# spcl/EBCC

Measured on AMD Instinct MI355X. Metric: fp32 GB/s encode+decode, 721x1440 ERA5 frames MAX_ERROR=0.5, higher is better.
Workload: dtype f32; 1 GPU; 256-frame batch 721x1440 fp32 per GPU, base_cr=30 MAX_ERROR=0.5 (BASELINE configs[1]); frames_per_gpu=256, parallelism=frames sharded over 1 GPU(s), no collective, hw_queues=4, encode_slices=3

## Files before the change

### ebcc_amd/csrc/j2k.hip

```cpp
#include <algorithm>
#include <cstring>
#include <vector>

#include "../../include/ebcc_hip.h"
#include "engine.hpp"
#include "j2k.hpp"

namespace ebcc {

bool j2k_create(ebcc_hip_ctx *ctx)
{
    J2kBuffers *jb = new J2kBuffers();
    ctx->j2k = jb;
    const int period = ctx->tile_period;
    std::vector<std::vector<J2kBlock>> tile_blocks((size_t) period);
    int stride = 0;
    for (int k = 0; k < period; k++) {
        jb->geoms.push_back(make_j2k_geom(ctx->height, ctx->width, tile_blocks[(size_t) k], k * ctx->height));
        stride = std::max(stride, jb->geoms.back().nblocks);
    }
    for (J2kGeom &t : jb->geoms) { t.period = period; t.stride = stride; }
    jb->geom = jb->geoms[0];
    const J2kGeom &g = jb->geom;
    const size_t n_pix = ctx->n_pix, F = ctx->max_frames;
// ... 19 lines not shown
    jb->SYM = nullptr;
    {
        const char *e = getenv("EBCC_T1_TWO_PHASE");
        jb->sym_rows = kJ2kSymRows;
        if (const char *r = getenv("EBCC_HIP_SYM_ROWS")) jb->sym_rows = std::max(1, std::min(kJ2kSymRows, atoi(r)));
        if (!e || atoi(e)) ok &= (jb->SYM = ctx_alloc<uint8_t>(ctx, groups * (size_t) ((jb->sym_rows + 1) & ~1) * 1024 + 256)) != nullptr;
    }
    ok &= (jb->seglen = ctx_alloc<uint16_t>(ctx, groups * (size_t) kJ2kSegCount * 64)) != nullptr;
    ok &= (jb->lanerows = ctx_alloc<uint32_t>(ctx, groups * 64)) != nullptr;
    ok &= (jb->qplane = (int *) ctx_alloc<int32_t>(ctx, groups * 64)) != nullptr;
    ok &= (jb->lastnp = (int *) ctx_alloc<int32_t>(ctx, groups * 64)) != nullptr;
    ok &= (jb->T1S = ctx_alloc<unsigned long long>(ctx, groups * kT1StateWords * 64)) != nullptr;
    ok &= (jb->blkmax = (int *) ctx_alloc<int32_t>(ctx, groups * 64)) != nullptr;
    ok &= (jb->numbps = (int *) ctx_alloc<int32_t>(ctx, groups * 64)) != nullptr;
    ok &= (jb->totalpasses = (int *) ctx_alloc<int32_t>(ctx, groups * 64)) != nullptr;
    ok &= (jb->cblk_len = (int *) ctx_alloc<int32_t>(ctx, groups * 64)) != nullptr;
    ok &= (jb->npass = (int *) ctx_alloc<int32_t>(ctx, groups * 64)) != nullptr;
    ok &= (jb->cand_cr = ctx_alloc<float>(ctx, F * 2)) != nullptr;
    ok &= (jb->cand_out = (int *) ctx_alloc<int32_t>(ctx, F * 6)) != nullptr;
    ok &= (jb->cand_npass = (int *) ctx_alloc<int32_t>(ctx, 2 * F * (size_t) stride)) != nullptr;
    ok &= (jb->cand_sel = (int *) ctx_alloc<int32_t>(ctx, F)) != nullptr;
    ok &= (jb->have_rate = (int *) ctx_alloc<int32_t>(ctx, F)) != nullptr;
    ok &= (jb->rate_path = (int *) ctx_alloc<int32_t>(ctx, F * 1536 * 3)) != nullptr;
    ok &= (jb->rate_path_n = (int *) ctx_alloc<int32_t>(ctx, 2 * F)) != nullptr;
    {
        int nodes = 0;
        for (const J2kGeom &t : jb->geoms) nodes = std::max(nodes, t.tree_nodes);
        J2kBuffers::RateCache &rc = jb->rate_cache;
        rc.nodes_cap = (nodes + 3) & ~3;
        rc.cap = stride * kJ2kMaxPasses;
        rc.ok = jb->rate_path_n ? jb->rate_path_n + F : nullptr;
        ok &= (rc.mnmx = ctx_alloc<double>(ctx, F * 2)) != nullptr;
        ok &= (rc.mval = (short *) ctx_alloc<uint16_t>(ctx, F * (size_t) rc.nodes_cap)) != nullptr;
        ok &= (rc.off = (int *) ctx_alloc<int32_t>(ctx, F * (size_t) (stride + 1))) != nullptr;
        ok &= (rc.crate = ctx_alloc<uint16_t>(ctx, F * (size_t) rc.cap)) != nullptr;
        ok &= (rc.cdisto = ctx_alloc<double>(ctx, F * (size_t) rc.cap)) != nullptr;
    }
    ok &= (jb->rates = (int *) ctx_alloc<int32_t>(ctx, groups * 64 * kJ2kMaxPasses)) != nullptr;
    ok &= (jb->disto = ctx_alloc<double>(ctx, groups * 64 * kJ2kMaxPasses)) != nullptr;
    ok &= (jb->cblk_bytes = ctx_alloc<uint8_t>(ctx, groups * 64 * kJ2kCblkBytes)) != nullptr;
    ok &= (jb->stream = ctx_alloc<uint8_t>(ctx, F * jb->stream_cap)) != nullptr;
    ok &= (jb->dec_table = (int *) ctx_alloc<int32_t>(ctx, groups * 64 * 4)) != nullptr;
    ok &= (jb->dec_order = (int *) ctx_alloc<int32_t>(ctx, groups * 64 + 128)) != nullptr;
    ok &= (jb->mq_order = (int *) ctx_alloc<int32_t>(ctx, groups * 64 + 256)) != nullptr;
    ok &= (jb->jf = (J2kFrame *) ctx_alloc<uint8_t>(ctx, sizeof(J2kFrame) * F)) != nullptr;
    ok &= (jb->partial = ctx_alloc<double>(ctx, F * kPartials)) != nullptr;
    ok &= (jb->partial_u = ctx_alloc<unsigned long long>(ctx, F * kPartials)) != nullptr;
    if (!ok) return false;
    poison_alloc(jb->cblk_bytes, groups * 64 * kJ2kCblkBytes);
    poison_alloc(jb->stream, F * jb->stream_cap);
    if (stride >= 65535) { set_error("too many code-blocks"); return false; }
    std::vector<uint16_t> map((size_t) period * n_pix, 0);
    std::vector<J2kBlock> blocks((size_t) period * (size_t) stride, J2kBlock{});
    for (int k = 0; k < period; k++) {
        const std::vector<J2kBlock> &tb = tile_blocks[(size_t) k];
        std::copy(tb.begin(), tb.end(), blocks.begin() + (size_t) k * (size_t) stride);
        for (size_t b = 0; b < tb.size(); b++)
            for (int y = 0; y < tb[b].h; y++)
                for (int x = 0; x < tb[b].w; x++) map[(size_t) k * n_pix + (size_t) (tb[b].y + y) * g.W + tb[b].x + x] = (uint16_t) b;
    }
    hipStream_t s = ctx->stream;
    EBCC_HIP_CHECK(hipMemcpyAsync(jb->d_geom, jb->geoms.data(), sizeof(J2kGeom) * (size_t) period, hipMemcpyHostToDevice, s));
    EBCC_HIP_CHECK(hipMemcpyAsync(jb->d_blocks, blocks.data(), sizeof(J2kBlock) * blocks.size(), hipMemcpyHostToDevice, s));
    EBCC_HIP_CHECK(hipMemcpyAsync(jb->d_blkmap, map.data(), map.size() * sizeof(uint16_t), hipMemcpyHostToDevice, s));
    EBCC_HIP_CHECK(hipHostMalloc(&ctx->h_jf, sizeof(J2kFrame) * F));
    EBCC_HIP_CHECK(hipHostMalloc((void **) &ctx->h_table, sizeof(int) * 4 * total));
    EBCC_HIP_CHECK(hipMemsetAsync(jb->jf, 0, sizeof(J2kFrame) * F, s));
    EBCC_HIP_CHECK(hipMemsetAsync(jb->rate_path_n, 0, sizeof(int) * 2 * F, s));
    wait_stream(s);
    return true;
}

void j2k_destroy(ebcc_hip_ctx *ctx)
{
    delete static_cast<J2kBuffers *>(ctx->j2k);
    ctx->j2k = nullptr;
    if (ctx->stream2) { hipStreamSynchronize(ctx->stream2); hipStreamDestroy(ctx->stream2); ctx->stream2 = nullptr; }
}

namespace {

struct BitReader {
    const uint8_t *p, *end;
    unsigned buf = 0;
    int ct = 0;
    int bit()
    {
        if (ct == 0) {
            buf = (buf << 8) & 0xFFFF;
            ct = buf == 0xFF00 ? 7 : 8;
            if (p < end) buf |= *p++;
// ... 470 lines not shown
```

### ebcc_amd/csrc/j2k.hpp

```cpp
#pragma once

#include <vector>

#include "../../include/ebcc_hip.h"
#include "common.hpp"
#include "residual.hpp"

namespace ebcc {

constexpr int kJ2kRes = 6;
constexpr int kJ2kBands = 3 * kJ2kRes - 2;
constexpr int kJ2kMaxPlanes = 26;
constexpr int kJ2kMaxPasses = 3 * kJ2kMaxPlanes;
constexpr int kJ2kCblkBytes = 16 * 1024;
constexpr int kT1StateWords = 66 + 4 * 64;

struct J2kBand {
    int res, orient, level;
    int x0, y0, x1, y1;
    int offx, offy;
    int ncw, nch;
    int first_block;
    int expn, mant, numbps;
    float step_enc, step_dec;
// ... 88 lines not shown
    unsigned long long *T1S;
    int *blkmax;
    int *numbps;
    int *totalpasses;
    int *cblk_len;
    int *rates;
    double *disto;
    int *npass;
    float *cand_cr;
    int *cand_out;
    int *cand_npass;
    int *cand_sel;
    int *have_rate;
    int *rate_path;
    int *rate_path_n;
    struct RateCache {
        int *ok;
        double *mnmx;
        short *mval;
        int *off;
        unsigned short *crate;
        double *cdisto;
        int nodes_cap, cap;
    } rate_cache;
    uint8_t *cblk_bytes;
    uint8_t *stream;
    size_t stream_cap;
    int32_t *V;
    int *dec_table;
    int *dec_order;
    int *mq_order;
    J2kFrame *jf;
    FrameState *fs;
    double *partial;
    unsigned long long *partial_u;
};

enum T1Kernel { T1_ENCODE = 0, T1_MQ = 1, T1_RESUME = 2, T1_DECODE = 3 };
int t1_lanes_per_wave(int kernel, int total_blocks = 0);

J2kGeom make_j2k_geom(int H, int W, std::vector<J2kBlock> &blocks, int ty0 = 0);

struct J2kWindow {
    int row0, col0, rows, cols;
    int rx0[kJ2kRes], rx1[kJ2kRes], ry0[kJ2kRes], ry1[kJ2kRes];
    int band[kJ2kBands][4];
// ... 58 lines not shown
```

### ebcc_amd/csrc/j2k_analysis.hip

```cpp
#include <array>
#include <mutex>
#include <cmath>
#include <cstdlib>
#include <vector>

#include "j2k.hpp"
#include "t1_core.hpp"
#include "t1_device.hpp"

namespace ebcc {

static int ceildivpow2(int a, int b) { return (int) (((long long) a + (1ll << b) - 1) >> b); }
static int floorlog2i(int a) { int l = 0; while (a > 1) { a >>= 1; l++; } return l; }

static const double kNormsReal[4][10] = {
    {1.000, 1.965, 4.177, 8.403, 16.90, 33.84, 67.69, 135.3, 270.6, 540.9},
    {2.022, 3.989, 8.355, 17.04, 34.27, 68.63, 137.3, 274.6, 549.0},
    {2.022, 3.989, 8.355, 17.04, 34.27, 68.63, 137.3, 274.6, 549.0},
    {2.080, 3.865, 8.307, 17.18, 34.71, 69.59, 139.3, 278.6, 557.2}};

int t1_lanes_per_wave(int kernel, int total_blocks)
{
    int t[4] = {64, 64, 4, 2};
    if (const char *e = getenv("EBCC_T1_LPW")) {
// ... 1101 lines not shown
};
__device__ inline Tier1Lane tier1_lane(int gid, int total, const int *blkmax, const J2kGeom *geom, const J2kBlock *blocks, const FrameState *fs)
{
    Tier1Lane l{gid, 0, 0, 0, 0, 0, false};
    if (gid >= total) return l;
    const int nb = geom->stride;
    l.frame = gid / nb;
    if (fs[l.frame].const_field) return l;
    const J2kBlock blk = j2k_frame_blocks(geom, blocks, l.frame)[gid - l.frame * nb];
    const int m = blkmax[gid];
    l.P = m ? (31 - __clz(m)) + 1 - 6 : 0;
    l.w = blk.w; l.h = blk.h;
    l.orient = j2k_frame_geom(geom, l.frame).bands[blk.band].orient;
    l.live = l.P > 0;
    return l;
}

struct ScanOutDev {
    unsigned char *vp, *sp;
    std::uint16_t *lens;
    uint32_t lane8;
    __device__ void visp_row(unsigned char *b, int row, unsigned long long v) const { *(unsigned long long *) (b + ((uint32_t) row * 512u + lane8)) = v; }
    __device__ void visp(int p, int y, unsigned long long m) const { visp_row(vp, p * 64 + y, m); }
    __device__ void sps_or(int y, unsigned long long n) const { *(unsigned long long *) (sp + ((uint32_t) y * 512u + lane8)) |= n; }
    __device__ void len(int seg, uint32_t n) const { lens[(uint32_t) seg * 64u] = (std::uint16_t) n; }
};
__global__ __launch_bounds__(64) void k_t1_scan(const unsigned long long *BP, const unsigned long long *SUF, const unsigned long long *SGN,
                                                 unsigned long long *SPS, unsigned long long *VISP, const int *blkmax, int *numbps,
                                                 int *totalpasses, int *cblk_len, std::uint16_t *seglen, const J2kGeom *geom,
                                                 const J2kBlock *blocks, const FrameState *fs, int total)
{
    const size_t grp = blockIdx.x;
    const int gid = (int) (grp * 64) + (int) threadIdx.x;
    const Tier1Lane l = tier1_lane(gid, total, blkmax, geom, blocks, fs);
    if (gid < total) { numbps[gid] = l.P; totalpasses[gid] = l.live ? 3 * l.P - 2 : 0; cblk_len[gid] = 0; }
    if (!l.live) return;
    const uint32_t lane8 = threadIdx.x * 8u;
    DevMasks M{(const unsigned char *) (BP + grp * kJ2kMaxPlanes * 64 * 64), (const unsigned char *) (SUF + grp * (kJ2kMaxPlanes + 2) * 64 * 64),
               (const unsigned char *) (SGN + grp * 64 * 64), (unsigned char *) (VISP + grp * kJ2kMaxPlanes * 64 * 64), lane8};
    ScanOutDev out{M.visp, (unsigned char *) (SPS + grp * 64 * 64), seglen + grp * kJ2kSegCount * 64 + threadIdx.x, lane8};
    t1::scan_block(M, out, l.P, l.w, l.h, l.orient);
}

__global__ __launch_bounds__(64) void k_t1_rowoffs(std::uint16_t *seglen, uint32_t *lanerows, const int *blkmax, J2kFrame *jf,
                                                    const J2kGeom *geom, const J2kBlock *blocks, const FrameState *fs, int total,
                                                    uint32_t sym_rows)
{
    const size_t grp = blockIdx.x;
    const int gid = (int) (grp * 64) + (int) threadIdx.x;
    const Tier1Lane l = tier1_lane(gid, total, blkmax, geom, blocks, fs);
    std::uint16_t *L = seglen + grp * kJ2kSegCount * 64 + threadIdx.x;
    uint32_t off = 0;
    if (l.live) {
        const int nstr = (l.h + 3) >> 2;
        for (int seg0 = t1::seg_index(l.P - 1, 2, 0) & ~15; seg0 < kJ2kSegCount; seg0 += 16) {
            if (!t1::seg_valid(l.P, nstr, t1::seg_plane(seg0), t1::seg_type(seg0), 0)) continue;
            uint32_t n[16];
#pragma unroll
            for (int k = 0; k < 16; k++) n[k] = k < nstr ? L[(uint32_t) (seg0 + k) * 64u] : 0u;
#pragma unroll
            for (int k = 0; k < 16; k++)
                if (k < nstr) { L[(uint32_t) (seg0 + k) * 64u] = (std::uint16_t) off; off += t1::seg_rows(n[k]); }
        }
    }
// ... 339 lines not shown
{
    const int f = blockIdx.x * blockDim.x + threadIdx.x;
    if (f < n) jf[f].overflow = 0;
}

void launch_j2k_tier1(const J2kBuffers &jb, int n_frames, hipStream_t s, bool single_kernel)
{
    const J2kGeom &g = jb.geom;
    const FrameState *fs = jb.fs;
    const int total = n_frames * g.stride;
    const size_t groups = ((size_t) total + 63) / 64;
    EBCC_HIP_CHECK(hipMemsetAsync(jb.SPS, 0, groups * 64 * 64 * sizeof(unsigned long long), s));
    timing_begin("t1_encode", s);
    if (!jb.SYM || single_kernel) {
        EBCC_HIP_CHECK(hipMemsetAsync(jb.T1S, 0, groups * kT1StateWords * 64 * sizeof(unsigned long long), s));
        int lpw = getenv("EBCC_T1_LPW") ? t1_lanes_per_wave(T1_ENCODE) : 32;
        unsigned t1_grid = (unsigned) ceil_div(total, lpw);
        hipLaunchKernelGGL(k_t1_encode, dim3(t1_grid), dim3(64), 0, s, jb.T1S, jb.BP, jb.SGN, jb.SPS, jb.blkmax, jb.numbps,
                           jb.totalpasses, jb.cblk_len, jb.rates, jb.cblk_bytes, jb.ckpt, jb.VISP, jb.d_geom,
                           jb.d_blocks, fs, jb.jf, total, lpw);
    } else {
        EBCC_HIP_CHECK(hipMemsetAsync(jb.seglen, 0, groups * (size_t) kJ2kSegCount * 64 * sizeof(std::uint16_t), s));
        timing_begin("t1_symbols", s);
        hipLaunchKernelGGL(k_t1_scan, dim3((unsigned) groups), dim3(64), 0, s, jb.BP, jb.SUF, jb.SGN, jb.SPS, jb.VISP, jb.blkmax, jb.numbps,
                           jb.totalpasses, jb.cblk_len, jb.seglen, jb.d_geom, jb.d_blocks, fs, total);
        hipLaunchKernelGGL(k_t1_rowoffs, dim3((unsigned) groups), dim3(64), 0, s, jb.seglen, jb.lanerows, jb.blkmax, jb.jf, jb.d_geom, jb.d_blocks,
                           fs, total, (uint32_t) jb.sym_rows);
        hipLaunchKernelGGL(k_t1_emit, dim3((unsigned) groups, kJ2kMaxPlanes), dim3(64), 0, s, jb.BP, jb.SUF, jb.SGN, jb.VISP, jb.blkmax, jb.SYM,
                           jb.seglen, jb.lanerows, jb.d_geom, jb.d_blocks, fs, total, (uint32_t) jb.sym_rows);
        timing_end("t1_symbols", s);
        if (getenv("EBCC_HIP_T1_STATS")) {
            std::vector<uint32_t> tot((size_t) total);
            EBCC_HIP_CHECK(hipMemcpyAsync(tot.data(), jb.lanerows, sizeof(uint32_t) * (size_t) total, hipMemcpyDeviceToHost, s));
            wait_stream(s);
            uint32_t mx = 0; double sum = 0, wsum = 0;
            for (size_t g0 = 0; g0 < (size_t) total; g0 += 64) {
                uint32_t wm = 0;
                for (size_t i = g0; i < std::min((size_t) total, g0 + 64); i++) { wm = std::max(wm, tot[i]); sum += tot[i]; }
                wsum += wm; mx = std::max(mx, wm);
            }
            fprintf(stderr, "ebcc-mi355x tier-1: %zu groups, rows of 16 decisions: per code-block mean %.0f, per wave mean %.0f max %u (cap %d)\n", groups,
                    sum / (double) total, wsum / (double) groups, mx, jb.sym_rows);
        }
        timing_begin("t1_mq", s);
        const int *order = nullptr;
        if (!getenv("EBCC_HIP_MQ_NATURAL_ORDER")) {
            int *counters = jb.mq_order + groups * 64;
// ... 65 lines not shown
            const float e2 = (i < dn) ? e1_2 + (((i == 0 ? o2 : o2_3) + o2) * kD) : e1_2 + ((2 * o2_3) * kD);
            b[(size_t) i * W] = e2 * invK;
            if (i < dn) b[(size_t) (sn + i) * W] = o2 * kK;
        }
        E_1 = E0; O_1 = O0;
        o1_2 = o1; e1_2 = e1;
        o2_3 = o2;
        e_in = e_nx; o_in = o_nx;
    }
}

void launch_j2k_analysis(const float *data, const J2kBuffers &jb, int n_frames, hipStream_t s)
{
    const FrameState *fs = jb.fs;
    const J2kGeom &g = jb.geom;
    const size_t n_pix = (size_t) g.W * g.H;
    const int total = n_frames * g.stride;
    hipLaunchKernelGGL(k_jf_reset, dim3(ceil_div(n_frames, 64)), dim3(64), 0, s, jb.jf, n_frames);
    const bool fwd_top = g.period == 1 && g.ry0[kJ2kRes - 1] % 2 == 0 && g.rh[kJ2kRes - 2] >= 2 &&
                         g.rh[kJ2kRes - 1] - g.rh[kJ2kRes - 2] >= 1;
    if (!fwd_top) hipLaunchKernelGGL(k_scale_shift, dim3(128, n_frames), dim3(256), 0, s, data, jb.B, n_pix, fs);
    EBCC_HIP_CHECK(hipMemsetAsync(jb.rate_path_n, 0, sizeof(int) * (size_t) n_frames, s));
    EBCC_HIP_CHECK(hipMemsetAsync(jb.rate_cache.ok, 0, sizeof(int) * (size_t) n_frames, s));
    EBCC_HIP_CHECK(hipMemsetAsync(jb.lastnp, 0xFF, sizeof(int) * (size_t) total, s));
    timing_begin("j2k_dwt_fwd", s);
    for (int r = kJ2kRes - 1; r >= 1; r--) {
        if (fwd_top && r == kJ2kRes - 1) {
            const int pieces = std::max(1, std::min(8, g.rh[r - 1] / 16));
            hipLaunchKernelGGL(k_j2k_cols_fwd_top, dim3(ceil_div(g.rw[r], kFwdT), n_frames, pieces), dim3(kFwdT), 0, s, data, jb.B, jb.d_geom, fs);
        } else
        dwt_cols<true>(jb.B, jb, r, n_frames, fs, nullptr, s);
        if (g.rw[r] > 1) dwt_rows<true>(jb.B, nullptr, jb, r, n_frames, fs, nullptr, s);
    }
    timing_end("j2k_dwt_fwd", s);
    hipLaunchKernelGGL(k_quantize, dim3((unsigned) (((size_t) total + 63) / 64)), dim3(256), 0, s, jb.B, jb.Q6, jb.BP, jb.SGN, jb.SUF, jb.blkmax,
                       jb.d_geom, jb.d_blocks, fs, total);
    launch_j2k_tier1(jb, n_frames, s, false);
    EBCC_HIP_LAUNCH_CHECK();
}

int j2k_first_fused(const J2kBuffers &jb)
{
    const J2kGeom &g = jb.geom;
    auto fusable = [&](int r) {
        return g.period == 1 && g.ry0[r] % 2 == 0 && g.rw[r - 1] >= 2 && g.rh[r - 1] >= 1 &&
               (r == kJ2kRes - 1 ? ceil_div(g.rw[r - 1], kL5Pairs) <= kPartials : jb.B2 != nullptr);
// ... 123 lines not shown
```

### ebcc_amd/csrc/j2k_rate.hip

```cpp
#include <cfloat>
#include <cmath>
#include <cstdlib>
#include <mutex>

#include "j2k.hpp"
#include "t1_core.hpp"
#include "t1_device.hpp"

namespace ebcc {

int j2k_inverse_dwt(float *B, const int32_t *V, const float *data, const J2kBuffers &jb, int n_frames, const FrameState *fs,
                    const int *active, hipStream_t s, int keep_field, const J2kWindow *win = nullptr, float *win_out = nullptr);

namespace {

constexpr int kMainHeaderBytes = 135;
constexpr int kRateTrieNodes = 1536;
#ifndef EBCC_RATE_THREADS
#define EBCC_RATE_THREADS 512
#endif
constexpr int kRateThreads = EBCC_RATE_THREADS;
constexpr int kWriteThreads = 256;

__device__ inline int floorlog2d(int a) { return a > 1 ? 31 - __clz(a) : 0; }
// ... 456 lines not shown
    }
    if (wl == 0) atomicAdd(s_sum, body + count);
    __syncthreads();
    const int total = *s_sum;
    __syncthreads();
    return total;
}

__global__ __launch_bounds__(kRateThreads) void k_rate(const int *__restrict__ numbps, const int *__restrict__ totalpasses,
                                                        const int *__restrict__ rates, const double *__restrict__ disto,
                                                        int *__restrict__ npass_out, const J2kGeom *geom, J2kFrame *jf,
                                                        const FrameState *fs, const int *active, int pass_capacity,
                                                        int *__restrict__ path_bytes, int *__restrict__ path_n,
                                                        const float *cand_cr, int *cand_out, size_t cand_stride, const int *have_rate,
                                                        J2kBuffers::RateCache cache)
{
    extern __shared__ unsigned char lds_raw[];
    __shared__ int s_sum, s_changed;
#ifdef EBCC_RATE_PROFILE
    const long long t_start = wall_clock64();
#endif
    __shared__ double s_min[kRateThreads / 64], s_max[kRateThreads / 64];
    __shared__ double s_td[5];
    __shared__ int s_ti[5], s_nun, s_list[64];
    const int frame = blockIdx.x, lane = threadIdx.x;
    if ((active && !active[frame]) || fs[frame].const_field) return;
    const bool candidate = cand_cr != nullptr;
    const int slot = candidate ? (int) blockIdx.y : 0;
    const float cr_in = candidate ? cand_cr[2 * frame + slot] : jf[frame].cr;
    if (candidate ? !(cr_in > 0.0f) : (have_rate && have_rate[frame])) return;
    if (candidate) npass_out += (size_t) slot * cand_stride;
    const bool record = !candidate;
    const J2kGeom &g = j2k_frame_geom(geom, frame);
    const int gid0 = frame * g.stride;
    RateLds L;
    L.carve(lds_raw, g.nblocks, g.tree_nodes);
#ifdef EBCC_RATE_PROFILE
    long long t_s[5] = {0, 0, 0, 0, 0};
    t_s[0] = wall_clock64() - t_start;
#endif
    __shared__ int s_cached;
    if (lane == 0) s_cached = __hip_atomic_load(&cache.ok[frame], __ATOMIC_ACQUIRE, __HIP_MEMORY_SCOPE_AGENT);
    __syncthreads();
    const bool cached = s_cached != 0;
    short *const c_mval = cache.mval + (size_t) frame * cache.nodes_cap;
    int *const c_off = cache.off + (size_t) frame * (size_t) (g.stride + 1);
    unsigned short *const c_rate = cache.crate + (size_t) frame * (size_t) cache.cap;
// ... 126 lines not shown
    if ((lane & 63) == 0) { s_min[lane >> 6] = mn; s_max[lane >> 6] = mx; }
    __syncthreads();
    for (int i = 0; i < kRateThreads / 64; i++) { mn = s_min[i] < mn ? s_min[i] : mn; mx = s_max[i] > mx ? s_max[i] : mx; }
    if (record) {
        __threadfence();
        __syncthreads();
        if (lane == 0) {
            cache.mnmx[2 * frame] = mn; cache.mnmx[2 * frame + 1] = mx;
            if (pt.lds) { __threadfence(); __hip_atomic_store(&cache.ok[frame], 1, __ATOMIC_RELEASE, __HIP_MEMORY_SCOPE_AGENT); }
        }
    }
    }

#ifdef EBCC_RATE_PROFILE
    long long t_setup = wall_clock64() - t_start, t_ml = 0, t_sz = 0, t_replay_end = 0, t_tail = 0, t_loop_end = 0; int n_it = 0, n_real = 0, n_replayed = 0, n_tail = 0;
#define RP_T0 const long long rp0 = wall_clock64()
#define RP_ADD(acc) acc += wall_clock64() - rp0
#else
#define RP_T0
#define RP_ADD(acc)
#endif
    double good = -1;
    bool converged = false;
    if (rate > 0.0f) {
        const long long maxlen = (long long) ceil((double) rate);
        double lo = mn, hi = mx, thresh = 0, stable = 0, prev = -1;
        bool lo_seen = false, hi_seen = false;
        int bytes_lo = 0, bytes_hi = 0;
        int *const trie = path_bytes + (size_t) frame * kRateTrieNodes * 3;
        const int known = path_n[frame];
        int n_nodes = known;
        int cur = known > 0 ? 0 : -1, parent = -1, pdir = 0;
        bool lo_from_rec = false, hi_from_rec = false;
        for (int i = 0; i < 128; i++) {
            thresh = (lo + hi) / 2;
            if (i > 0 && thresh == prev) break;
            prev = thresh;
            if (cur >= 0) {
#ifdef EBCC_RATE_PROFILE
                n_replayed++;
#endif
                const int bytes = trie[3 * cur];
                const int f = (long long) bytes <= maxlen;
                if (f) { hi = thresh; stable = thresh; bytes_hi = bytes; hi_from_rec = true; hi_seen = false; }
                else { lo = thresh; bytes_lo = bytes; lo_from_rec = true; lo_seen = false; }
                parent = cur; pdir = f;
                const int nxt = trie[3 * cur + 1 + f];
                cur = nxt > 0 ? nxt : -1;
                continue;
            }
#ifdef EBCC_RATE_PROFILE
            if (!t_replay_end) t_replay_end = wall_clock64();
#endif
            if (hi_from_rec) { make_layer<kRateThreads>(g, L, totalpasses, pt, gid0, hi, lane, p_hi); hi_seen = true; hi_from_rec = false; }
            if (lo_from_rec) { make_layer<kRateThreads>(g, L, totalpasses, pt, gid0, lo, lane, p_lo); lo_seen = true; lo_from_rec = false; }
            { RP_T0; make_layer<kRateThreads>(g, L, totalpasses, pt, gid0, thresh, lane, p_cur, frozen); RP_ADD(t_ml); }
            if (lane == 0) s_nun = 0;
            int at_lo = lo_seen, at_hi = hi_seen;
            for (int b = lane; b < g.nblocks; b += kRateThreads) {
                if (frozen[b]) continue;
                if (p_cur[b] != p_lo[b] || p_cur[g.nblocks + b] != p_lo[g.nblocks + b]) at_lo = 0;
                if (p_cur[b] != p_hi[b] || p_cur[g.nblocks + b] != p_hi[g.nblocks + b]) at_hi = 0;
            }
            at_lo = __syncthreads_and(at_lo);
            at_hi = __syncthreads_and(at_hi);
            int bytes;
            if (at_lo) bytes = bytes_lo;
            else if (at_hi) bytes = bytes_hi;
            else { RP_T0; bytes = sized(); RP_ADD(t_sz); }
#ifdef EBCC_RATE_PROFILE
            n_it++; n_real += (at_lo || at_hi) ? 0 : s_changed;
#endif
            const bool fits = (long long) bytes <= maxlen;
            if (record && n_nodes < kRateTrieNodes && (parent >= 0 || n_nodes == 0)) {
                if (lane == 0) {
                    trie[3 * n_nodes] = bytes; trie[3 * n_nodes + 1] = 0; trie[3 * n_nodes + 2] = 0;
                    if (parent >= 0) trie[3 * parent + 1 + pdir] = n_nodes;
                    path_n[frame] = n_nodes + 1;
                }
                parent = n_nodes++; pdir = fits;
            } else {
                parent = -1;
            }
            if (fits) bytes_hi = bytes; else bytes_lo = bytes;
            if (fits) { hi = thresh; stable = thresh; hi_seen = true; } else { lo = thresh; lo_seen = true; }
            unsigned long long *end = fits ? p_hi : p_lo;
            int same = lo_seen && hi_seen;
            for (int b = lane; b < g.nblocks; b += kRateThreads) {
                if (frozen[b]) continue;
                end[b] = p_cur[b]; end[g.nblocks + b] = p_cur[g.nblocks + b];
                if (lo_seen && hi_seen && p_lo[b] == p_hi[b] && p_lo[g.nblocks + b] == p_hi[g.nblocks + b]) frozen[b] = 1;
                else {
                    same = 0;
                    const int k = atomicAdd(&s_nun, 1);
                    if (k < 64) s_list[k] = b;
                }
            }
            if (__syncthreads_and(same)) { converged = true; break; }
            if (lo_seen && hi_seen && s_nun <= 64) {
                RP_T0;
                if (lane < 64) {
                    const int nb = g.nblocks, b = lane < s_nun ? s_list[lane] : -1;
                    double tlo = lo, thi = hi, tprev = prev, tstable = stable, tthresh = thresh;
                    int ti = i, tn = n_nodes, tparent = parent, tpdir = pdir, status = 0;
                    int from = 0, n_in = 0;
                    unsigned long long c0 = 0, c1 = 0;
                    if (b >= 0) {
                        const unsigned long long d0 = p_lo[b] ^ p_hi[b], d1 = p_lo[nb + b] ^ p_hi[nb + b];
                        from = d0 ? __builtin_ctzll(d0) : (d1 ? 64 + __builtin_ctzll(d1) : 0);
                        if (from > 0) {
                            c0 = from >= 64 ? p_lo[b] : p_lo[b] & ((1ull << from) - 1ull);
                            c1 = from > 64 ? p_lo[nb + b] & ((1ull << (from - 64)) - 1ull) : 0ull;
                            n_in = c1 ? 128 - __builtin_clzll(c1) : (c0 ? 64 - __builtin_clzll(c0) : 0);
                        }
                    }
                    double a_lo = -DBL_MAX, b_lo = DBL_MAX, a_hi = -DBL_MAX, b_hi = DBL_MAX;
                    if (b >= 0) {
                        if (pt.lds) {
                            walk_interval<true>(pt, totalpasses, gid0, b, p_lo[b], p_lo[nb + b], from, n_in, tlo, thi, a_lo, b_lo);
                            walk_interval<true>(pt, totalpasses, gid0, b, p_hi[b], p_hi[nb + b], from, n_in, tlo, thi, a_hi, b_hi);
                        } else {
                            walk_interval<false>(pt, totalpasses, gid0, b, p_lo[b], p_lo[nb + b], from, n_in, tlo, thi, a_lo, b_lo);
                            walk_interval<false>(pt, totalpasses, gid0, b, p_hi[b], p_hi[nb + b], from, n_in, tlo, thi, a_hi, b_hi);
                        }
                    }
                    (void) c0; (void) c1;
                    for (int j = i + 1; j < 128; j++) {
                        const double t = (tlo + thi) / 2;
                        if (t == tprev) { tthresh = t; break; }
                        const int all_lo = __all(b < 0 || (t >= a_lo && t < b_lo));
                        const int all_hi = __all(b < 0 || (t >= a_hi && t < b_hi));
                        if (!all_lo && !all_hi) { status = 1; break; }
                        tthresh = t; tprev = t; ti = j;
                        const int bytes = all_lo ? bytes_lo : bytes_hi;
                        const bool fits = (long long) bytes <= maxlen;
                        if (record && tn < kRateTrieNodes && (tparent >= 0 || tn == 0)) {
                            if (lane == 0) {
                                trie[3 * tn] = bytes; trie[3 * tn + 1] = 0; trie[3 * tn + 2] = 0;
                                if (tparent >= 0) trie[3 * tparent + 1 + tpdir] = tn;
                                path_n[frame] = tn + 1;
                            }
                            tparent = tn++; tpdir = fits;
                        } else {
                            tparent = -1;
                        }
                        if (fits) { thi = t; tstable = t; } else { tlo = t; }
                    }
                    if (lane == 0) {
                        s_td[0] = tlo; s_td[1] = thi; s_td[2] = tprev; s_td[3] = tstable; s_td[4] = tthresh;
                        s_ti[0] = ti; s_ti[1] = tn; s_ti[2] = tparent; s_ti[3] = tpdir; s_ti[4] = status;
                    }
                }
                __syncthreads();
                lo = s_td[0]; hi = s_td[1]; prev = s_td[2]; stable = s_td[3]; thresh = s_td[4];
                i = s_ti[0]; n_nodes = s_ti[1]; parent = s_ti[2]; pdir = s_ti[3];
                const int status = s_ti[4];
                __syncthreads();
                RP_ADD(t_tail);
#ifdef EBCC_RATE_PROFILE
                n_tail++;
#endif
                if (status == 0) break;
            }
        }
        good = stable == 0 ? thresh : stable;
    }
#ifdef EBCC_RATE_PROFILE
    t_loop_end = wall_clock64();
#endif
    if (!converged) make_layer<kRateThreads>(g, L, totalpasses, pt, gid0, good, lane);
    const int body = sized();
    for (int b = lane; b < g.nblocks; b += kRateThreads) npass_out[gid0 + b] = L.npass[b];
    if (lane == 0 && candidate) {
        int *o = cand_out + (size_t) (2 * frame + slot) * 3;
        o[0] = body; o[1] = kMainHeaderBytes + 12 + 2 + body + 2; o[2] = (int) (rate > 0.0f ? ceil((double) rate) : 0);
    }
    if (lane == 0 && !candidate) {
        jf[frame].body_bytes = body;
        jf[frame].stream_bytes = kMainHeaderBytes + 12 + 2 + body + 2;
        jf[frame].maxlen = (int) (rate > 0.0f ? ceil((double) rate) : 0);
#ifdef EBCC_RATE_PROFILE
        if (frame == 0) printf("k_rate frame0 setup: entry %lld, trees %lld, offsets %lld, tables %lld us\n", t_s[0] / 100, t_s[1] / 100, t_s[2] / 100, t_s[3] / 100);
        if (frame == 0) printf("k_rate frame0: setup %lld us, %d replayed steps until %lld us, make_layer %lld us, sized %lld us, computed iterations %d (real sizings %d), tail %lld us in %d visits, loop ends at %lld us, total %lld us\n",
                               t_setup / 100, n_replayed, t_replay_end ? (t_replay_end - t_start) / 100 : -1, t_ml / 100, t_sz / 100, n_it, n_real, t_tail / 100, n_tail,
                               (t_loop_end - t_start) / 100, (wall_clock64() - t_start) / 100);
#endif
    }
}

__device__ inline void put16(uint8_t *&p, unsigned v) { *p++ = (uint8_t) (v >> 8); *p++ = (uint8_t) v; }
__device__ inline void put32(uint8_t *&p, unsigned v) { put16(p, v >> 16); put16(p, v & 0xFFFFu); }

__global__ __launch_bounds__(kWriteThreads) void k_write(const int *__restrict__ numbps, const int *__restrict__ rates,
                                                         const int *__restrict__ npass_in, const uint8_t *__restrict__ cblk_bytes,
                                                         uint8_t *__restrict__ stream, size_t stream_cap, const J2kGeom *geom,
                                                         J2kFrame *jf, const FrameState *fs, const int *active)
{
    extern __shared__ unsigned char lds_raw[];
    __shared__ int s_hdr[kJ2kRes], s_body[kJ2kRes], s_off[kJ2kRes + 1];
    const int frame = blockIdx.x, lane = threadIdx.x;
    if ((active && !active[frame]) || fs[frame].const_field) return;
    const J2kGeom &g = j2k_frame_geom(geom, frame);
    const int gid0 = frame * g.stride;
    RateLds L;
    L.carve(lds_raw, g.nblocks, g.tree_nodes);
    trees_static<kWriteThreads>(g, L, numbps, gid0, lane);
    for (int b = lane; b < g.nblocks; b += kWriteThreads) L.npass[b] = (short) npass_in[gid0 + b];
    __syncthreads();
// ... 749 lines not shown
```

### ebcc_amd/csrc/t1_core.hpp

```cpp
#pragma once

#include <cstdint>
#include <type_traits>

#if defined(__HIPCC__)
#define T1_HD __host__ __device__ inline
#else
#define T1_HD inline
#endif
#ifndef T1_STAT
#define T1_STAT(i)
#endif

namespace ebcc {
namespace t1 {

typedef unsigned long long u64;

enum { CTX_ZC0 = 0, CTX_SC0 = 9, CTX_MAG0 = 14, CTX_AGG = 17, CTX_UNI = 18, NCTX = 19 };
constexpr int kMaxPasses = 3 * 30;

T1_HD uint32_t mq_entry(int i)
{
    constexpr uint32_t T[47] = {
// ... 1144 lines not shown
    r.length = n;
    return r;
}

constexpr int kSegPlanes = 26;
constexpr int kSegCount = kSegPlanes * 3 * 16;
T1_HD int seg_index(int p, int t, int s) { return ((kSegPlanes - 1 - p) * 3 + t) * 16 + s; }
T1_HD int seg_plane(int seg) { return kSegPlanes - 1 - seg / 48; }
T1_HD int seg_type(int seg) { return (seg >> 4) % 3; }
T1_HD bool seg_valid(int P, int nstr, int p, int t, int s) { return p < P && (p < P - 1 || t == 2) && s < nstr; }

template <class Masks>
struct MaskRows {
    Masks &M;
    int h;
    T1_HD u64 bp(int p, int y) const { return (y >= 0 && y < h) ? M.BP(p, y) : 0ull; }
    T1_HD u64 suf(int p, int y) const { return (y >= 0 && y < h) ? M.SUF(p, y) : 0ull; }
    T1_HD u64 sgn(int y) const { return (y >= 0 && y < h) ? M.SGN(y) : 0ull; }
    T1_HD u64 visp(int p, int y) const { return (y >= 0 && y < h) ? M.VISP(p, y) : 0ull; }
};
struct NullCoder {};

template <class Masks, class Out>
T1_HD void scan_block(Masks &M, Out &out, int P, int w, int h, int orient)
{
    NullCoder nc;
    Passes<true, Masks, NullCoder> ps(M, nc, w, h, orient);
    const MaskRows<Masks> R{M, h};
    const int nstr = (h + 3) >> 2;
    for (int p = P - 1; p >= 0; p--) {
        const bool top = p == P - 1;
        Stripe sp;
        sp.wmask = w >= 64 ? ~0ull : ((1ull << w) - 1);
        if (!top) {
            u64 carry = 0;
            for (int s = 0; s < nstr; s++) {
                const int y0 = 4 * s;
                sp.nrows = h - y0 < 4 ? h - y0 : 4;
#pragma unroll
                for (int r = 0; r < 6; r++) sp.s[r] = R.suf(p + 1, y0 - 1 + r);
                const u64 b[4] = {R.bp(p, y0), R.bp(p, y0 + 1), R.bp(p, y0 + 2), R.bp(p, y0 + 3)};
                const uint32_t nref = (uint32_t) (ps.popc64(sp.s[1]) + ps.popc64(sp.s[2]) + ps.popc64(sp.s[3]) + ps.popc64(sp.s[4]));
                sp.s[0] |= carry;
                u64 m[4], n[4];
                ps.sigprop_members(sp, b, m, n);
#pragma unroll
                for (int r = 0; r < 4; r++)
                    if (r < sp.nrows) { out.visp(p, y0 + r, m[r]); if (n[r]) out.sps_or(y0 + r, n[r]); }
                out.len(seg_index(p, 0, s), ps.sigprop_count(m, n));
                out.len(seg_index(p, 1, s), nref);
                carry = n[3];
            }
        }
        for (int s = 0; s < nstr; s++) {
            const int y0 = 4 * s;
            sp.nrows = h - y0 < 4 ? h - y0 : 4;
            sp.s[0] = R.suf(p, y0 - 1);
#pragma unroll
            for (int r = 1; r < 6; r++) {
                const int y = y0 - 1 + r;
                sp.s[r] = R.suf(p + 1, y) | (top ? 0ull : (R.visp(p, y) & R.bp(p, y)));
            }
#pragma unroll
            for (int r = 0; r < 4; r++) sp.vis[r] = top ? 0ull : R.visp(p, y0 + r);
            const u64 b[4] = {R.bp(p, y0), R.bp(p, y0 + 1), R.bp(p, y0 + 2), R.bp(p, y0 + 3)};
            u64 m[4], n[4], agg;
            ps.cleanup_members(sp, b, y0 + 3 < h, m, n, agg);
            out.len(seg_index(p, 2, s), ps.cleanup_count(m, n, b, agg));
        }
    }
}

template <class Masks, class Em>
T1_HD void emit_stripe_segments(Masks &M, Em &em, int P, int p, int s, int w, int h, int orient)
{
    Passes<true, Masks, Em> ps(M, em, w, h, orient);
    const MaskRows<Masks> R{M, h};
    const bool top = p == P - 1;
    const int y0 = 4 * s;
    u64 s1[6], A[6], sg[6], vp[6];
#pragma unroll
    for (int r = 0; r < 6; r++) {
        const int y = y0 - 1 + r;
        s1[r] = R.suf(p + 1, y);
        sg[r] = R.sgn(y);
        vp[r] = top ? 0ull : R.visp(p, y);
        A[r] = s1[r] | (vp[r] & R.bp(p, y));
    }
    const u64 b[4] = {R.bp(p, y0), R.bp(p, y0 + 1), R.bp(p, y0 + 2), R.bp(p, y0 + 3)};
    Stripe sp;
    sp.wmask = w >= 64 ? ~0ull : ((1ull << w) - 1);
    sp.nrows = h - y0 < 4 ? h - y0 : 4;
#pragma unroll
// ... 263 lines not shown
```

Measured before the change: 8.905 GB/s.

## Parallelize tier-1 scan across bit-planes and memoize rate-control final layers

The tier-1 symbol scan kernel now launches one grid row per bit-plane, so each plane of a code-block is scanned independently. Because planes now share the same SPS rows, the updates to SPS use atomicOr. The rate-control epilogue also avoids recomputing the final layer and its size. It reuses the npass bracket masks and byte counts already known from the search, and keeps a small per-frame memo keyed by threshold for repeated candidate evaluations. The costs are more launched blocks, most of which exit early, extra atomics, and extra memory and fences for the memo.

```diff
diff --git a/ebcc_amd/csrc/j2k.hip b/ebcc_amd/csrc/j2k.hip
--- a/ebcc_amd/csrc/j2k.hip
+++ b/ebcc_amd/csrc/j2k.hip
@@ -65,7 +65,7 @@
     ok &= (jb->cand_sel = (int *) ctx_alloc<int32_t>(ctx, F)) != nullptr;
     ok &= (jb->have_rate = (int *) ctx_alloc<int32_t>(ctx, F)) != nullptr;
     ok &= (jb->rate_path = (int *) ctx_alloc<int32_t>(ctx, F * 1536 * 3)) != nullptr;
-    ok &= (jb->rate_path_n = (int *) ctx_alloc<int32_t>(ctx, 2 * F)) != nullptr;
+    ok &= (jb->rate_path_n = (int *) ctx_alloc<int32_t>(ctx, 3 * F)) != nullptr;
     {
         int nodes = 0;
         for (const J2kGeom &t : jb->geoms) nodes = std::max(nodes, t.tree_nodes);
@@ -73,6 +73,11 @@
         rc.nodes_cap = (nodes + 3) & ~3;
         rc.cap = stride * kJ2kMaxPasses;
         rc.ok = jb->rate_path_n ? jb->rate_path_n + F : nullptr;
+        rc.memo_n = jb->rate_path_n ? jb->rate_path_n + 2 * F : nullptr;
+        rc.memo_stride = stride;
+        ok &= (rc.memo_key = ctx_alloc<unsigned long long>(ctx, F * J2kBuffers::RateCache::kMemo)) != nullptr;
+        ok &= (rc.memo_body = (int *) ctx_alloc<int32_t>(ctx, F * J2kBuffers::RateCache::kMemo)) != nullptr;
+        ok &= (rc.memo_npass = ctx_alloc<uint8_t>(ctx, F * J2kBuffers::RateCache::kMemo * (size_t) stride)) != nullptr;
         ok &= (rc.mnmx = ctx_alloc<double>(ctx, F * 2)) != nullptr;
         ok &= (rc.mval = (short *) ctx_alloc<uint16_t>(ctx, F * (size_t) rc.nodes_cap)) != nullptr;
         ok &= (rc.off = (int *) ctx_alloc<int32_t>(ctx, F * (size_t) (stride + 1))) != nullptr;
@@ -109,7 +114,7 @@
     EBCC_HIP_CHECK(hipHostMalloc(&ctx->h_jf, sizeof(J2kFrame) * F));
     EBCC_HIP_CHECK(hipHostMalloc((void **) &ctx->h_table, sizeof(int) * 4 * total));
     EBCC_HIP_CHECK(hipMemsetAsync(jb->jf, 0, sizeof(J2kFrame) * F, s));
-    EBCC_HIP_CHECK(hipMemsetAsync(jb->rate_path_n, 0, sizeof(int) * 2 * F, s));
+    EBCC_HIP_CHECK(hipMemsetAsync(jb->rate_path_n, 0, sizeof(int) * 3 * F, s));
     wait_stream(s);
     return true;
 }
diff --git a/ebcc_amd/csrc/j2k.hpp b/ebcc_amd/csrc/j2k.hpp
--- a/ebcc_amd/csrc/j2k.hpp
+++ b/ebcc_amd/csrc/j2k.hpp
@@ -134,6 +134,12 @@
         unsigned short *crate;
         double *cdisto;
         int nodes_cap, cap;
+        static constexpr int kMemo = 8;
+        int *memo_n;
+        unsigned long long *memo_key;
+        int *memo_body;
+        unsigned char *memo_npass;
+        int memo_stride;
     } rate_cache;
     uint8_t *cblk_bytes;
     uint8_t *stream;
diff --git a/ebcc_amd/csrc/j2k_analysis.hip b/ebcc_amd/csrc/j2k_analysis.hip
--- a/ebcc_amd/csrc/j2k_analysis.hip
+++ b/ebcc_amd/csrc/j2k_analysis.hip
@@ -1147,7 +1147,7 @@
     uint32_t lane8;
     __device__ void visp_row(unsigned char *b, int row, unsigned long long v) const { *(unsigned long long *) (b + ((uint32_t) row * 512u + lane8)) = v; }
     __device__ void visp(int p, int y, unsigned long long m) const { visp_row(vp, p * 64 + y, m); }
-    __device__ void sps_or(int y, unsigned long long n) const { *(unsigned long long *) (sp + ((uint32_t) y * 512u + lane8)) |= n; }
+    __device__ void sps_or(int y, unsigned long long n) const { atomicOr((unsigned long long *) (sp + ((uint32_t) y * 512u + lane8)), n); }
     __device__ void len(int seg, uint32_t n) const { lens[(uint32_t) seg * 64u] = (std::uint16_t) n; }
 };
 __global__ __launch_bounds__(64) void k_t1_scan(const unsigned long long *BP, const unsigned long long *SUF, const unsigned long long *SGN,
@@ -1156,15 +1156,16 @@
                                                  const J2kBlock *blocks, const FrameState *fs, int total)
 {
     const size_t grp = blockIdx.x;
+    const int p = (int) blockIdx.y;
     const int gid = (int) (grp * 64) + (int) threadIdx.x;
     const Tier1Lane l = tier1_lane(gid, total, blkmax, geom, blocks, fs);
-    if (gid < total) { numbps[gid] = l.P; totalpasses[gid] = l.live ? 3 * l.P - 2 : 0; cblk_len[gid] = 0; }
-    if (!l.live) return;
+    if (p == 0 && gid < total) { numbps[gid] = l.P; totalpasses[gid] = l.live ? 3 * l.P - 2 : 0; cblk_len[gid] = 0; }
+    if (!l.live || p >= l.P) return;
     const uint32_t lane8 = threadIdx.x * 8u;
     DevMasks M{(const unsigned char *) (BP + grp * kJ2kMaxPlanes * 64 * 64), (const unsigned char *) (SUF + grp * (kJ2kMaxPlanes + 2) * 64 * 64),
                (const unsigned char *) (SGN + grp * 64 * 64), (unsigned char *) (VISP + grp * kJ2kMaxPlanes * 64 * 64), lane8};
     ScanOutDev out{M.visp, (unsigned char *) (SPS + grp * 64 * 64), seglen + grp * kJ2kSegCount * 64 + threadIdx.x, lane8};
-    t1::scan_block(M, out, l.P, l.w, l.h, l.orient);
+    t1::scan_plane(M, out, l.P, p, l.w, l.h, l.orient);
 }
 
 __global__ __launch_bounds__(64) void k_t1_rowoffs(std::uint16_t *seglen, uint32_t *lanerows, const int *blkmax, J2kFrame *jf,
@@ -1550,7 +1551,7 @@
     } else {
         EBCC_HIP_CHECK(hipMemsetAsync(jb.seglen, 0, groups * (size_t) kJ2kSegCount * 64 * sizeof(std::uint16_t), s));
         timing_begin("t1_symbols", s);
-        hipLaunchKernelGGL(k_t1_scan, dim3((unsigned) groups), dim3(64), 0, s, jb.BP, jb.SUF, jb.SGN, jb.SPS, jb.VISP, jb.blkmax, jb.numbps,
+        hipLaunchKernelGGL(k_t1_scan, dim3((unsigned) groups, kJ2kMaxPlanes), dim3(64), 0, s, jb.BP, jb.SUF, jb.SGN, jb.SPS, jb.VISP, jb.blkmax, jb.numbps,
                            jb.totalpasses, jb.cblk_len, jb.seglen, jb.d_geom, jb.d_blocks, fs, total);
         hipLaunchKernelGGL(k_t1_rowoffs, dim3((unsigned) groups), dim3(64), 0, s, jb.seglen, jb.lanerows, jb.blkmax, jb.jf, jb.d_geom, jb.d_blocks,
                            fs, total, (uint32_t) jb.sym_rows);
@@ -1662,6 +1663,7 @@
     if (!fwd_top) hipLaunchKernelGGL(k_scale_shift, dim3(128, n_frames), dim3(256), 0, s, data, jb.B, n_pix, fs);
     EBCC_HIP_CHECK(hipMemsetAsync(jb.rate_path_n, 0, sizeof(int) * (size_t) n_frames, s));
     EBCC_HIP_CHECK(hipMemsetAsync(jb.rate_cache.ok, 0, sizeof(int) * (size_t) n_frames, s));
+    EBCC_HIP_CHECK(hipMemsetAsync(jb.rate_cache.memo_n, 0, sizeof(int) * (size_t) n_frames, s));
     EBCC_HIP_CHECK(hipMemsetAsync(jb.lastnp, 0xFF, sizeof(int) * (size_t) total, s));
     timing_begin("j2k_dwt_fwd", s);
     for (int r = kJ2kRes - 1; r >= 1; r--) {
diff --git a/ebcc_amd/csrc/j2k_rate.hip b/ebcc_amd/csrc/j2k_rate.hip
--- a/ebcc_amd/csrc/j2k_rate.hip
+++ b/ebcc_amd/csrc/j2k_rate.hip
@@ -502,7 +502,7 @@
 #endif
     __shared__ double s_min[kRateThreads / 64], s_max[kRateThreads / 64];
     __shared__ double s_td[5];
-    __shared__ int s_ti[5], s_nun, s_list[64];
+    __shared__ int s_ti[9], s_nun, s_list[64];
     const int frame = blockIdx.x, lane = threadIdx.x;
     if ((active && !active[frame]) || fs[frame].const_field) return;
     const bool candidate = cand_cr != nullptr;
@@ -675,6 +675,8 @@
 #endif
     double good = -1;
     bool converged = false;
+    int stable_bytes = -1, last_bytes = -1, stable_at = 0, last_at = 0;
+    int good_bytes = -1, good_at = 0;
     if (rate > 0.0f) {
         const long long maxlen = (long long) ceil((double) rate);
         double lo = mn, hi = mx, thresh = 0, stable = 0, prev = -1;
@@ -695,8 +697,9 @@
 #endif
                 const int bytes = trie[3 * cur];
                 const int f = (long long) bytes <= maxlen;
-                if (f) { hi = thresh; stable = thresh; bytes_hi = bytes; hi_from_rec = true; hi_seen = false; }
+                if (f) { hi = thresh; stable = thresh; bytes_hi = bytes; hi_from_rec = true; hi_seen = false; stable_bytes = bytes; stable_at = 0; }
                 else { lo = thresh; bytes_lo = bytes; lo_from_rec = true; lo_seen = false; }
+                last_bytes = bytes; last_at = 0;
                 parent = cur; pdir = f;
                 const int nxt = trie[3 * cur + 1 + f];
                 cur = nxt > 0 ? nxt : -1;
@@ -705,7 +708,10 @@
 #ifdef EBCC_RATE_PROFILE
             if (!t_replay_end) t_replay_end = wall_clock64();
 #endif
-            if (hi_from_rec) { make_layer<kRateThreads>(g, L, totalpasses, pt, gid0, hi, lane, p_hi); hi_seen = true; hi_from_rec = false; }
+            if (hi_from_rec) {
+                make_layer<kRateThreads>(g, L, totalpasses, pt, gid0, hi, lane, p_hi); hi_seen = true; hi_from_rec = false;
+                if (stable == hi) stable_at = 2;
+            }
             if (lo_from_rec) { make_layer<kRateThreads>(g, L, totalpasses, pt, gid0, lo, lane, p_lo); lo_seen = true; lo_from_rec = false; }
             { RP_T0; make_layer<kRateThreads>(g, L, totalpasses, pt, gid0, thresh, lane, p_cur, frozen); RP_ADD(t_ml); }
             if (lane == 0) s_nun = 0;
@@ -737,6 +743,8 @@
             }
             if (fits) bytes_hi = bytes; else bytes_lo = bytes;
             if (fits) { hi = thresh; stable = thresh; hi_seen = true; } else { lo = thresh; lo_seen = true; }
+            last_bytes = bytes; last_at = fits ? 2 : 1;
+            if (fits) { stable_bytes = bytes; stable_at = 2; } else if (stable_at == 1) stable_at = 0;
             unsigned long long *end = fits ? p_hi : p_lo;
             int same = lo_seen && hi_seen;
             for (int b = lane; b < g.nblocks; b += kRateThreads) {
@@ -756,6 +764,7 @@
                     const int nb = g.nblocks, b = lane < s_nun ? s_list[lane] : -1;
                     double tlo = lo, thi = hi, tprev = prev, tstable = stable, tthresh = thresh;
                     int ti = i, tn = n_nodes, tparent = parent, tpdir = pdir, status = 0;
+                    int t_sb = stable_bytes, t_lb = last_bytes, t_sa = stable_at, t_la = last_at;
                     int from = 0, n_in = 0;
                     unsigned long long c0 = 0, c1 = 0;
                     if (b >= 0) {
@@ -798,16 +807,20 @@
                             tparent = -1;
                         }
                         if (fits) { thi = t; tstable = t; } else { tlo = t; }
+                        t_lb = bytes; t_la = all_lo ? 1 : 2;
+                        if (fits) { t_sb = bytes; t_sa = t_la; }
                     }
                     if (lane == 0) {
                         s_td[0] = tlo; s_td[1] = thi; s_td[2] = tprev; s_td[3] = tstable; s_td[4] = tthresh;
                         s_ti[0] = ti; s_ti[1] = tn; s_ti[2] = tparent; s_ti[3] = tpdir; s_ti[4] = status;
+                        s_ti[5] = t_sb; s_ti[6] = t_lb; s_ti[7] = t_sa; s_ti[8] = t_la;
                     }
                 }
                 __syncthreads();
                 lo = s_td[0]; hi = s_td[1]; prev = s_td[2]; stable = s_td[3]; thresh = s_td[4];
                 i = s_ti[0]; n_nodes = s_ti[1]; parent = s_ti[2]; pdir = s_ti[3];
                 const int status = s_ti[4];
+                stable_bytes = s_ti[5]; last_bytes = s_ti[6]; stable_at = s_ti[7]; last_at = s_ti[8];
                 __syncthreads();
                 RP_ADD(t_tail);
 #ifdef EBCC_RATE_PROFILE
@@ -817,12 +830,75 @@
             }
         }
         good = stable == 0 ? thresh : stable;
+        good_bytes = stable == 0 ? last_bytes : stable_bytes;
+        good_at = good >= 0 ? (stable == 0 ? last_at : stable_at) : 0;
     }
 #ifdef EBCC_RATE_PROFILE
     t_loop_end = wall_clock64();
 #endif
-    if (!converged) make_layer<kRateThreads>(g, L, totalpasses, pt, gid0, good, lane);
-    const int body = sized();
+    constexpr int kMemo = J2kBuffers::RateCache::kMemo;
+    unsigned long long *const m_key = cache.memo_key + (size_t) frame * kMemo;
+    int *const m_body = cache.memo_body + (size_t) frame * kMemo;
+    unsigned char *const m_npass = cache.memo_npass + (size_t) frame * kMemo * (size_t) cache.memo_stride;
+    const unsigned long long key = (unsigned long long) __double_as_longlong(good);
+    __shared__ int s_memo[2];
+    if (lane < 64) {
+        const int n = __hip_atomic_load(&cache.memo_n[frame], __ATOMIC_ACQUIRE, __HIP_MEMORY_SCOPE_AGENT);
+        const bool match = lane < (n < kMemo ? n : kMemo) && __hip_atomic_load(&m_key[lane], __ATOMIC_ACQUIRE, __HIP_MEMORY_SCOPE_AGENT) == key;
+        const unsigned long long m = __ballot(match);
+        if (lane == 0) { s_memo[0] = m ? __ffsll((long long) m) - 1 : -1; s_memo[1] = n; }
+    }
+    __syncthreads();
+    const int memo_hit = s_memo[0], memo_count = s_memo[1];
+    int body;
+    if (memo_hit >= 0) {
+        for (int b = lane; b < g.nblocks; b += kRateThreads) L.npass[b] = (short) m_npass[(size_t) memo_hit * cache.memo_stride + b];
+        body = m_body[memo_hit];
+        __syncthreads();
+    } else {
+        if (converged) {
+        } else if (good_at) {
+            const unsigned long long *const pm = good_at == 1 ? p_lo : p_hi;
+            for (int b = lane; b < g.nblocks; b += kRateThreads) {
+                if (frozen[b]) continue;
+                const unsigned long long m0 = pm[b], m1 = pm[g.nblocks + b];
+                L.npass[b] = (short) (m1 ? 128 - __builtin_clzll(m1) : (m0 ? 64 - __builtin_clzll(m0) : 0));
+            }
+            __syncthreads();
+        } else {
+            make_layer<kRateThreads>(g, L, totalpasses, pt, gid0, good, lane);
+        }
+        body = good_bytes >= 0 ? good_bytes : sized();
+    }
+#ifdef EBCC_RATE_CHECK
+    {
+        for (int b = lane; b < g.nblocks; b += kRateThreads) L.prev[b] = L.npass[b];
+        __syncthreads();
+        make_layer<kRateThreads>(g, L, totalpasses, pt, gid0, good, lane);
+        const int ref = layer_bytes<kRateThreads>(g, L, rates, gid0, lane, &s_sum);
+        int bad = 0;
+        for (int b = lane; b < g.nblocks; b += kRateThreads) if (L.prev[b] != L.npass[b]) bad++;
+        bad = __syncthreads_count(bad);
+        if ((bad || ref != body) && lane == 0)
+            printf("rate check: frame %d epilogue (memo %d, converged %d, end %d): %d code-blocks differ, body %d serial %d\n", frame, memo_hit,
+                   (int) converged, good_at, bad, body, ref);
+        body = ref;
+    }
+#endif
+    if (record && memo_hit < 0) {
+        const int ms = memo_count % kMemo;
+        if (lane == 0) __hip_atomic_store(&m_key[ms], ~0ull, __ATOMIC_RELAXED, __HIP_MEMORY_SCOPE_AGENT);
+        __threadfence();
+        __syncthreads();
+        for (int b = lane; b < g.nblocks; b += kRateThreads) m_npass[(size_t) ms * cache.memo_stride + b] = (unsigned char) L.npass[b];
+        if (lane == 0) m_body[ms] = body;
+        __threadfence();
+        __syncthreads();
+        if (lane == 0) {
+            __hip_atomic_store(&m_key[ms], key, __ATOMIC_RELEASE, __HIP_MEMORY_SCOPE_AGENT);
+            __hip_atomic_store(&cache.memo_n[frame], memo_count + 1, __ATOMIC_RELEASE, __HIP_MEMORY_SCOPE_AGENT);
+        }
+    }
     for (int b = lane; b < g.nblocks; b += kRateThreads) npass_out[gid0 + b] = L.npass[b];
     if (lane == 0 && candidate) {
         int *o = cand_out + (size_t) (2 * frame + slot) * 3;
@@ -834,9 +910,9 @@
         jf[frame].maxlen = (int) (rate > 0.0f ? ceil((double) rate) : 0);
 #ifdef EBCC_RATE_PROFILE
         if (frame == 0) printf("k_rate frame0 setup: entry %lld, trees %lld, offsets %lld, tables %lld us\n", t_s[0] / 100, t_s[1] / 100, t_s[2] / 100, t_s[3] / 100);
-        if (frame == 0) printf("k_rate frame0: setup %lld us, %d replayed steps until %lld us, make_layer %lld us, sized %lld us, computed iterations %d (real sizings %d), tail %lld us in %d visits, loop ends at %lld us, total %lld us\n",
+        if (frame == 0) printf("k_rate frame0: setup %lld us, %d replayed steps until %lld us, make_layer %lld us, sized %lld us, computed iterations %d (real sizings %d), tail %lld us in %d visits, loop ends at %lld us, total %lld us (epilogue: memo slot %d, converged %d, bracket end %d, size known %d)\n",
                                t_setup / 100, n_replayed, t_replay_end ? (t_replay_end - t_start) / 100 : -1, t_ml / 100, t_sz / 100, n_it, n_real, t_tail / 100, n_tail,
-                               (t_loop_end - t_start) / 100, (wall_clock64() - t_start) / 100);
+                               (t_loop_end - t_start) / 100, (wall_clock64() - t_start) / 100, memo_hit, (int) converged, good_at, (int) (good_bytes >= 0));
 #endif
     }
 }
diff --git a/ebcc_amd/csrc/t1_core.hpp b/ebcc_amd/csrc/t1_core.hpp
--- a/ebcc_amd/csrc/t1_core.hpp
+++ b/ebcc_amd/csrc/t1_core.hpp
@@ -1190,53 +1190,56 @@
 struct NullCoder {};
 
 template <class Masks, class Out>
-T1_HD void scan_block(Masks &M, Out &out, int P, int w, int h, int orient)
+T1_HD void scan_plane(Masks &M, Out &out, int P, int p, int w, int h, int orient)
 {
     NullCoder nc;
     Passes<true, Masks, NullCoder> ps(M, nc, w, h, orient);
     const MaskRows<Masks> R{M, h};
     const int nstr = (h + 3) >> 2;
-    for (int p = P - 1; p >= 0; p--) {
-        const bool top = p == P - 1;
-        Stripe sp;
-        sp.wmask = w >= 64 ? ~0ull : ((1ull << w) - 1);
-        if (!top) {
-            u64 carry = 0;
-            for (int s = 0; s < nstr; s++) {
-                const int y0 = 4 * s;
-                sp.nrows = h - y0 < 4 ? h - y0 : 4;
-#pragma unroll
-                for (int r = 0; r < 6; r++) sp.s[r] = R.suf(p + 1, y0 - 1 + r);
-                const u64 b[4] = {R.bp(p, y0), R.bp(p, y0 + 1), R.bp(p, y0 + 2), R.bp(p, y0 + 3)};
-                const uint32_t nref = (uint32_t) (ps.popc64(sp.s[1]) + ps.popc64(sp.s[2]) + ps.popc64(sp.s[3]) + ps.popc64(sp.s[4]));
-                sp.s[0] |= carry;
-                u64 m[4], n[4];
-                ps.sigprop_members(sp, b, m, n);
-#pragma unroll
-                for (int r = 0; r < 4; r++)
-                    if (r < sp.nrows) { out.visp(p, y0 + r, m[r]); if (n[r]) out.sps_or(y0 + r, n[r]); }
-                out.len(seg_index(p, 0, s), ps.sigprop_count(m, n));
-                out.len(seg_index(p, 1, s), nref);
-                carry = n[3];
-            }
-        }
+    const bool top = p == P - 1;
+    Stripe sp;
+    sp.wmask = w >= 64 ? ~0ull : ((1ull << w) - 1);
+    if (!top) {
+        u64 carry = 0;
         for (int s = 0; s < nstr; s++) {
             const int y0 = 4 * s;
             sp.nrows = h - y0 < 4 ? h - y0 : 4;
-            sp.s[0] = R.suf(p, y0 - 1);
-#pragma unroll
-            for (int r = 1; r < 6; r++) {
-                const int y = y0 - 1 + r;
-                sp.s[r] = R.suf(p + 1, y) | (top ? 0ull : (R.visp(p, y) & R.bp(p, y)));
-            }
-#pragma unroll
-            for (int r = 0; r < 4; r++) sp.vis[r] = top ? 0ull : R.visp(p, y0 + r);
+#pragma unroll
+            for (int r = 0; r < 6; r++) sp.s[r] = R.suf(p + 1, y0 - 1 + r);
             const u64 b[4] = {R.bp(p, y0), R.bp(p, y0 + 1), R.bp(p, y0 + 2), R.bp(p, y0 + 3)};
-            u64 m[4], n[4], agg;
-            ps.cleanup_members(sp, b, y0 + 3 < h, m, n, agg);
-            out.len(seg_index(p, 2, s), ps.cleanup_count(m, n, b, agg));
-        }
-    }
+            const uint32_t nref = (uint32_t) (ps.popc64(sp.s[1]) + ps.popc64(sp.s[2]) + ps.popc64(sp.s[3]) + ps.popc64(sp.s[4]));
+            sp.s[0] |= carry;
+            u64 m[4], n[4];
+            ps.sigprop_members(sp, b, m, n);
+#pragma unroll
+            for (int r = 0; r < 4; r++)
+                if (r < sp.nrows) { out.visp(p, y0 + r, m[r]); if (n[r]) out.sps_or(y0 + r, n[r]); }
+            out.len(seg_index(p, 0, s), ps.sigprop_count(m, n));
+            out.len(seg_index(p, 1, s), nref);
+            carry = n[3];
+        }
+    }
+    for (int s = 0; s < nstr; s++) {
+        const int y0 = 4 * s;
+        sp.nrows = h - y0 < 4 ? h - y0 : 4;
+        sp.s[0] = R.suf(p, y0 - 1);
+#pragma unroll
+        for (int r = 1; r < 6; r++) {
+            const int y = y0 - 1 + r;
+            sp.s[r] = R.suf(p + 1, y) | (top ? 0ull : (R.visp(p, y) & R.bp(p, y)));
+        }
+#pragma unroll
+        for (int r = 0; r < 4; r++) sp.vis[r] = top ? 0ull : R.visp(p, y0 + r);
+        const u64 b[4] = {R.bp(p, y0), R.bp(p, y0 + 1), R.bp(p, y0 + 2), R.bp(p, y0 + 3)};
+        u64 m[4], n[4], agg;
+        ps.cleanup_members(sp, b, y0 + 3 < h, m, n, agg);
+        out.len(seg_index(p, 2, s), ps.cleanup_count(m, n, b, agg));
+    }
+}
+template <class Masks, class Out>
+T1_HD void scan_block(Masks &M, Out &out, int P, int w, int h, int orient)
+{
+    for (int p = P - 1; p >= 0; p--) scan_plane(M, out, P, p, w, h, orient);
 }
 
 template <class Masks, class Em>
```

After: 8.995 GB/s, median of 6. About the same (+1.0%).
